# jontio/JAERO

Hardware: AMD Instinct MI355X
Metric: Msamples/s of real 48 kHz PCM through the 10.5 kbps OQPSK demodulator hot path (higher is better)
Workload: dtype f64; 1 GPU; 65536-channel-per-GPU synthetic 48 kHz 10.5 kbps OQPSK continuous (BASELINE configs[2] shape, scaled to 65536 channels per GPU = one wavefront of 64 channels per SIMD), 4096-sample writes, coarse 2^14 FFT every 4096 samples, AFC off, EbNo meters on, Eb/N0 10.0 dB, per-channel carrier (8000 +- 100 Hz), bits, noise, symbol phase; 42 untimed pre-roll steps (the last 18 resident and back to back with ; channels_per_gpu=65536, total_channels=65536, chunk=4096, ebno_meters=True, preroll_steps=42, timing_phases=32, hbm_bytes_per_resident_channel=2256640, resident_channels_max=137027, ranks=1, control_plane=none (single rank), sustain_steps=18

## Files before the change

### jaero_amd/csrc/jaero_device.h

```cpp
#pragma once
#include <hip/hip_runtime.h>
#include <stdint.h>
#include "jd_libm.h"

#define JD_WTSIZE 19999
#define JD_WAVE 64

enum
{
    S_M2_PTR, S_M2_STEP, S_M2_FREQ,
    S_MC_PTR, S_MC_STEP, S_MC_FREQ,
    S_ST_PTR, S_ST_STEP, S_ST_FREQ, S_ST_LAST,
    S_AGC_SUM,
    S_EB_ESUM, S_EB_E2SUM, S_EB_EBNO,
    S_D1,
    S_D41_1, S_D41_2, S_D41_3,
    S_D42_1, S_D42_2, S_D42_3,
    S_D8_1, S_D8_2,
    S_RES_X1, S_RES_X2, S_RES_Y1, S_RES_Y2,
    S_LF_X1, S_LF_X2, S_LF_Y1, S_LF_Y2,
    S_SIG2L_RE, S_SIG2L_IM, S_PTD_RE, S_PTD_IM,
    S_MARG_SUM, S_PM_SUM, S_MSEMA_SUM, S_MSE,
    S_DIFF_LAST,
    S_LOCKINGBW, S_THRESH,
// ... 411 lines not shown
                if (((hx & 0xfffffu) | (unsigned)__double2loint(x)) != 0) return x + x;
                return (xsb == 0) ? x : -1.0;
            }
            if (x > o_threshold) return huge * huge;
        }
        if (xsb != 0 && x + tiny < 0.0) return tiny - one;
    }
    if (hx > 0x3fd62e42u)
    {
        if (hx < 0x3FF0A2B2u)
        {
            if (xsb == 0) { hi = x - ln2_hi; lo = ln2_lo; k = 1; }
            else { hi = x + ln2_hi; lo = -ln2_lo; k = -1; }
        }
        else
        {
            k = (int)(invln2 * x + ((xsb == 0) ? 0.5 : -0.5));
            t = k;
            hi = x - t * ln2_hi;
            lo = t * ln2_lo;
        }
        x = hi - lo;
        c = (hi - x) - lo;
    }
    else if (hx < 0x3c900000u) return x;
    else k = 0;
    hfx = 0.5 * x;
    hxs = x * hfx;
    {
        const double R1 = one + hxs * Q1, h2 = hxs * hxs;
        const double R2 = Q2 + hxs * Q3, h4 = h2 * h2;
        const double R3 = Q4 + hxs * Q5;
        r1 = R1 + h2 * R2 + h4 * R3;
    }
    t = 3.0 - r1 * hfx;
    e = hxs * ((r1 - t) / (6.0 - x * t));
    if (k == 0) return x - (x * e - hxs);
    e = (x * (e - c) - c);
    e -= hxs;
    if (k == -1) return 0.5 * (x - e) - 0.5;
    if (k == 1)
    {
        if (x < -0.25) return -2.0 * (e - (x + 0.5));
        return one + 2.0 * (x - e);
    }
    if (k <= -2 || k > 56)
    {
        y = one - (e - x);
        y = jd_with_hi(y, __double2hiint(y) + (k << 20));
        return y - one;
    }
    if (k < 20)
    {
        t = jd_with_hi(one, 0x3ff00000 - (0x200000 >> k));
        y = t - (e - x);
        y = jd_with_hi(y, __double2hiint(y) + (k << 20));
    }
    else
    {
        t = jd_with_hi(one, (0x3ff - k) << 20);
        y = x - (e + t);
        y += one;
        y = jd_with_hi(y, __double2hiint(y) + (k << 20));
    }
    return y;
}
__device__ __noinline__ double jd_tanh_full(double x)
{
    const double one = 1.0, two = 2.0, tiny = 1.0e-300;
    double t, z;
    const int jx = __double2hiint(x);
    const int ix = jx & 0x7fffffff;
    if (ix >= 0x7ff00000) return (jx >= 0) ? one / x + one : one / x - one;
    if (ix < 0x40360000)
    {
        if ((ix | __double2loint(x)) == 0) return x;
        if (ix < 0x3c800000) return x * (one + x);
        const bool big = ix >= 0x3ff00000;
        const double ax2 = two * fabs(x);
        t = jd_expm1(big ? ax2 : -ax2);
        const double q = (big ? two : t) / (t + two);
        z = big ? one - q : -q;
    }
    else z = one - tiny;
    return (jx >= 0) ? z : -z;
}

__device__ __forceinline__ double jd_tanh(double xin)
{
    const double one = 1.0, two = 2.0, ln2_hi = 6.93147180369123816490e-01, ln2_lo = 1.90821492927058770002e-10,
                 invln2 = 1.44269504088896338700e+00, Q1 = -3.33333333333331316428e-02, Q2 = 1.58730158725481460165e-03,
                 Q3 = -7.93650757867487942473e-05, Q4 = 4.00821782732936239552e-06, Q5 = -2.01099218183624371326e-07;
    const int jx = __double2hiint(xin), ix = jx & 0x7fffffff;
    if (!(ix >= 0x3c800000 && ix < 0x401a0000)) return jd_tanh_full(xin);
    const bool big = ix >= 0x3ff00000;
    const double ax2 = two * fabs(xin);
    double x = big ? ax2 : -ax2;
    const unsigned hx = (unsigned)__double2hiint(x) & 0x7fffffffu;
    const int k = (hx > 0x3fd62e42u) ? (int)(invln2 * x + (big ? 0.5 : -0.5)) : 0;
    const double tk = (double)k;
    const double hi = x - tk * ln2_hi, lo = tk * ln2_lo;
    x = hi - lo;
    const double c = (hi - x) - lo;
    const double hfx = 0.5 * x, hxs = x * hfx;
    const double R1 = one + hxs * Q1, h2 = hxs * hxs, R2 = Q2 + hxs * Q3, h4 = h2 * h2, R3 = Q4 + hxs * Q5;
    const double r1 = R1 + h2 * R2 + h4 * R3;
    const double t3 = 3.0 - r1 * hfx;
    const double e = hxs * jd_div(r1 - t3, 6.0 - x * t3);
    const double r_k0 = x - (x * e - hxs);
    double e2 = (x * (e - c) - c);
    e2 -= hxs;
    const double r_m1 = 0.5 * (x - e2) - 0.5;
    double yn = one - (e2 - x);
    yn = jd_with_hi(yn, __double2hiint(yn) + (k << 20));
    const double r_neg = yn - one;
    const double tm = jd_with_hi(one, 0x3ff00000 - (0x200000 >> (k & 31)));
    double ym = tm - (e2 - x);
    ym = jd_with_hi(ym, __double2hiint(ym) + (k << 20));
    const double t = (k == 0) ? r_k0 : (k == -1) ? r_m1 : (k <= -2) ? r_neg : ym;
    const double q = jd_div(big ? two : t, t + two);
    const double z = big ? one - q : -q;
    return (jx >= 0) ? z : -z;
}

__device__ __forceinline__ double jd_log10(double x)
{
#pragma clang fp contract(fast)
    int e;
    double m = frexp(x, &e);
    if (m < 0.70710678118654752440) { m *= 2.0; e -= 1; }
    const double d = m + 1.0, n = m - 1.0;
    double r = __builtin_amdgcn_rcp(d);
    r = fma(fma(-d, r, 1.0), r, r);
    r = fma(fma(-d, r, 1.0), r, r);
    const double s = n * r;
    const double sl = fma(-d, s, n) * r;
    const double z = s * s;
    double q = 1.0 / 19.0;
    q = fma(q, z, 1.0 / 17.0);
    q = fma(q, z, 1.0 / 15.0);
    q = fma(q, z, 1.0 / 13.0);
    q = fma(q, z, 1.0 / 11.0);
    q = fma(q, z, 1.0 / 9.0);
    q = fma(q, z, 1.0 / 7.0);
    q = fma(q, z, 1.0 / 5.0);
    q = fma(q, z, 1.0 / 3.0);
    const double t = fma(s * z, q, sl);
    const double kh = 0x1.bcb7b1526e50ep-1, kl = 0x1.95355baaafad3p-56;
    const double ch = 0x1.34413509f79ffp-2, cl = -0x1.9dc1da994fd21p-59;
    const double u = fma(s, kh, fma(t, kh, s * kl));
    const double ef = (double)e;
    return fma(ef, ch, fma(ef, cl, u));
}
```

### jaero_amd/csrc/k_coarse6.h

```cpp
#pragma once
#include "k_coarse2.h"

#ifndef C4_TABN
#define C4_TABN 3584
#endif
#define C6_FENCE __builtin_amdgcn_sched_barrier(0)
__device__ __forceinline__ double2 c6_sq(const double2 a)
{
#pragma clang fp contract(fast)
    return make_double2(a.x * a.x - a.y * a.y, 2.0 * (a.x * a.y));
}

#ifndef C6_TRACE
#define C6_TRACE(i)
#endif

template <int CTRL, int ROWMASK>
__device__ __forceinline__ void c6_argmax_step(double &bv, int &bi)
{
    const int lo = __builtin_amdgcn_update_dpp(__double2loint(bv), __double2loint(bv), CTRL, ROWMASK, 0xf, false);
    const int hi = __builtin_amdgcn_update_dpp(__double2hiint(bv), __double2hiint(bv), CTRL, ROWMASK, 0xf, false);
    const int oi = __builtin_amdgcn_update_dpp(bi, bi, CTRL, ROWMASK, 0xf, false);
    const double ov = __hiloint2double(hi, lo);
    const bool take = (oi >= 0) & ((bi < 0) | (ov > bv) | ((ov == bv) & (oi < bi)));
    bv = take ? ov : bv;
    bi = take ? oi : bi;
}
__device__ __forceinline__ void c6_wave_argmax(double &bv, int &bi)
{
    c6_argmax_step<0xB1, 0xf>(bv, bi);
    c6_argmax_step<0x4E, 0xf>(bv, bi);
    c6_argmax_step<0x141, 0xf>(bv, bi);
    c6_argmax_step<0x140, 0xf>(bv, bi);
    c6_argmax_step<0x142, 0xa>(bv, bi);
    c6_argmax_step<0x143, 0xc>(bv, bi);
    bv = __hiloint2double(__builtin_amdgcn_readlane(__double2hiint(bv), 63), __builtin_amdgcn_readlane(__double2loint(bv), 63));
    bi = __builtin_amdgcn_readlane(bi, 63);
}

#define C6_XCH 16448

__device__ __forceinline__ constexpr int c6_k(int s) { return s < 16 ? 2 * s : 2 * (s - 16) + 1; }

__device__ __forceinline__ void c6_fft32(CV<32> &x)
{
#pragma clang fp contract(fast)
#pragma unroll
    for (int j = 0; j < 16; j++)
    {
        const double ar = x.r[j], ai = x.i[j], br = x.r[j + 16], bi = x.i[j + 16];
        x.r[j] = ar + br; x.i[j] = ai + bi;
        double dr = ar - br, di = ai - bi;
        cmul_w64(dr, di, 2 * j);
        x.r[j + 16] = dr; x.i[j + 16] = di;
    }
    C6_FENCE;
#pragma unroll
    for (int h = 0; h < 2; h++)
    {
        CV<16> in, out;
#pragma unroll
        for (int j = 0; j < 16; j++) { in.r[j] = x.r[16 * h + j]; in.i[j] = x.i[16 * h + j]; }
        regfft<16>(in, out);
#pragma unroll
        for (int j = 0; j < 16; j++) { x.r[16 * h + j] = out.r[j]; x.i[16 * h + j] = out.i[j]; }
        C6_FENCE;
    }
}

__device__ __forceinline__ void c6_twiddle32(CV<32> &x, const double2 p1)
{
#pragma clang fp contract(fast)
    auto app = [&](int slot, const double2 w) __attribute__((always_inline)) {
        const double r = x.r[slot] * w.x - x.i[slot] * w.y, i = x.r[slot] * w.y + x.i[slot] * w.x;
        x.r[slot] = r; x.i[slot] = i;
    };
    const double2 p2 = c6_sq(p1);
    double2 e = p2;
    app(16, p1);
#pragma unroll
    for (int j = 1; j < 16; j++)
    {
        app(j, e);
        app(16 + j, cmul2(e, p1));
        if (j < 15) e = cmul2(e, p2);
    }
}

#ifndef C6_ABSORB
#define C6_ABSORB 2
#endif

__device__ __forceinline__ constexpr int c6_brev(int v, int bits)
{
    int r = 0;
    for (int i = 0; i < bits; i++) r |= ((v >> i) & 1) << (bits - 1 - i);
    return r;
}

__device__ __forceinline__ double2 c6_root_mul(const double2 p, int idx)
{
#pragma clang fp contract(fast)
    const int e = idx & 15;
    double2 r = p;
    if (e != 0)
    {
        const double wr = jd_w64r(e), wi = jd_w64i(e);
        r = make_double2(p.x * wr - p.y * wi, p.x * wi + p.y * wr);
    }
    return (idx & 16) ? make_double2(r.y, -r.x) : r;
}

__device__ __forceinline__ void c6_ratio_powers(const double2 r, double2 (&P)[5])
{
    P[0] = r;
#pragma unroll
    for (int i = 1; i < 5; i++) P[i] = c6_sq(P[i - 1]);
}

template <int L, int OFF, int Z>
__device__ __forceinline__ void c6_afft(CV<32> &x, const double2 (&P)[5])
{
    constexpr int LG = L == 32 ? 5 : 4, S = 64 / L;
#pragma unroll
    for (int lv = 0; lv < LG; lv++)
    {
#pragma unroll
        for (int b = 0; b < (1 << lv); b++)
        {
            const int half = L >> (lv + 1);
            const double2 w = c6_root_mul(P[LG - 1 - lv], half * (S * c6_brev(b, lv) + Z));
#pragma unroll
            for (int j = 0; j < half; j++)
            {
                const int ia = OFF + 2 * half * b + j, ib = ia + half;
                const double ar = x.r[ia], ai = x.i[ia], br = x.r[ib], bi = x.i[ib];
                const double ur = __builtin_fma(-w.y, bi, __builtin_fma(w.x, br, ar));
                const double ui = __builtin_fma(w.x, bi, __builtin_fma(w.y, br, ai));
                x.r[ia] = ur; x.i[ia] = ui;
                x.r[ib] = __builtin_fma(2.0, ar, -ur); x.i[ib] = __builtin_fma(2.0, ai, -ui);
            }
        }
        C6_FENCE;
    }
}

__device__ __forceinline__ void c6_afft16x2(CV<32> &x, const double2 r)
{
    double2 P[5];
    c6_ratio_powers(r, P);
    c6_afft<16, 0, 0>(x, P);
    c6_afft<16, 16, 2>(x, P);
}

template <int L, int OFF>
__device__ __forceinline__ void c6_twiddle_brev(CV<32> &x, const double2 c, const double2 s)
{
#pragma clang fp contract(fast)
    constexpr int LG = L == 32 ? 5 : 4;
    auto app = [&](int slot, const double2 w) __attribute__((always_inline)) {
        const double r = x.r[slot] * w.x - x.i[slot] * w.y, i = x.r[slot] * w.y + x.i[slot] * w.x;
        x.r[slot] = r; x.i[slot] = i;
    };
    const double2 s2 = c6_sq(s);
    double2 e = c;
#pragma unroll
    for (int j = 0; j < L / 2; j++)
    {
        app(OFF + c6_brev(2 * j, LG), e);
        app(OFF + c6_brev(2 * j + 1, LG), cmul2(e, s));
        if (j < L / 2 - 1) e = cmul2(e, s2);
    }
}

template <bool ABSORBED>
__device__ __forceinline__ void c6_pass3(CV<32> &d, const double2 r)
{
    if constexpr (ABSORBED)
    {
        c6_afft16x2(d, r);
        const CV<32> o = d;
#pragma unroll
        for (int k3 = 0; k3 < 16; k3++)
        {
            d.r[2 * k3] = o.r[c6_brev(k3, 4)]; d.i[2 * k3] = o.i[c6_brev(k3, 4)];
            d.r[2 * k3 + 1] = o.r[16 + c6_brev(k3, 4)]; d.i[2 * k3 + 1] = o.i[16 + c6_brev(k3, 4)];
        }
    }
    else
    {
        CV<16> in, o0, o1;
#pragma unroll
        for (int j = 0; j < 16; j++) { in.r[j] = d.r[j]; in.i[j] = d.i[j]; }
        regfft<16>(in, o0);
        C6_FENCE;
#pragma unroll
        for (int j = 0; j < 16; j++) { in.r[j] = d.r[16 + j]; in.i[j] = d.i[16 + j]; }
        regfft<16>(in, o1);
#pragma unroll
        for (int k3 = 0; k3 < 16; k3++) { d.r[2 * k3] = o0.r[k3]; d.i[2 * k3] = o0.i[k3]; d.r[2 * k3 + 1] = o1.r[k3]; d.i[2 * k3 + 1] = o1.i[k3]; }
    }
}

template <int AB = C6_ABSORB>
__device__ __forceinline__ void wg_fft14_e32(CV<32> &d, double *xch, const double2 *__restrict__ tw, int t)
{
#pragma clang fp contract(fast)
    const int k1u = t >> 4, n3 = t & 15, odd = k1u & 1;
    const double2 st1 = tw[AB ? 16 * k1u : t], st2 = tw[AB == 2 ? t : 32 * n3];
    double2 st3 = st2;
    if constexpr (AB == 1) st3 = tw[k1u * n3];
    const int e1w0 = t, e1w1 = (t + 16) & 511;
    const int e1r = k1u * 512 + odd * 16 + n3;
    const int e1rw = e1r + 496 - 512 * odd;
    const int e2w = k1u + n3 * 513;
    const int e2r = t;
    auto k2of = [](int s) __attribute__((always_inline)) { return AB ? c6_brev(s, 5) : c6_k(s); };

    c6_fft32(d);
    if constexpr (AB == 0) c6_twiddle32(d, st1);
    C6_FENCE;
    jd_lds_barrier();
#pragma unroll
    for (int s = 0; s < 32; s++) xch[c6_k(s) * 512 + ((c6_k(s) & 1) ? e1w1 : e1w0)] = d.r[s];
    jd_lds_barrier();
#pragma unroll
    for (int m = 0; m < 32; m++) d.r[m] = xch[(m < 31 ? e1r + 16 * m : e1rw)];
    jd_lds_barrier();
#pragma unroll
    for (int s = 0; s < 32; s++) xch[c6_k(s) * 512 + ((c6_k(s) & 1) ? e1w1 : e1w0)] = d.i[s];
    jd_lds_barrier();
#pragma unroll
    for (int m = 0; m < 32; m++) d.i[m] = xch[(m < 31 ? e1r + 16 * m : e1rw)];
    C6_FENCE;
    if constexpr (AB == 0)
    {
        c6_fft32(d);
        c6_twiddle32(d, st2);
    }
    else
    {
        double2 P[5];
        c6_ratio_powers(st1, P);
        c6_afft<32, 0, 0>(d, P);
        if constexpr (AB == 1) c6_twiddle_brev<32, 0>(d, st3, st2);
    }
    C6_FENCE;
    jd_lds_barrier();
#pragma unroll
    for (int s = 0; s < 32; s++) xch[e2w + (k2of(s) & 15) * 32 + (k2of(s) >> 4) * 8208] = d.r[s];
    jd_lds_barrier();
#pragma unroll
    for (int m = 0; m < 32; m++) d.r[m] = xch[e2r + (m & 15) * 513 + (m >> 4) * 8208];
    jd_lds_barrier();
#pragma unroll
    for (int s = 0; s < 32; s++) xch[e2w + (k2of(s) & 15) * 32 + (k2of(s) >> 4) * 8208] = d.i[s];
    jd_lds_barrier();
#pragma unroll
    for (int m = 0; m < 32; m++) d.i[m] = xch[e2r + (m & 15) * 513 + (m >> 4) * 8208];
    C6_FENCE;
    c6_pass3<AB == 2>(d, st2);
}


#define C6_XCH13 8208
template <int AB = C6_ABSORB>
__device__ __forceinline__ void wg_fft13_e32(CV<32> &d, double *xch, const double2 *__restrict__ tw, int t)
{
#pragma clang fp contract(fast)
    const int k1a = t >> 4, n3 = t & 15;
    const double2 st1 = tw[AB ? 16 * k1a : t], st2 = tw[AB == 2 ? t : 32 * n3];
    const int e1r = k1a * 256 + n3;
    const int e2w = k1a + 513 * n3;
    auto k2of = [](int s) __attribute__((always_inline)) { return AB ? c6_brev(s & 15, 4) : (s & 15); };
    c6_fft32(d);
    if constexpr (AB == 0) c6_twiddle32(d, st1);
    C6_FENCE;
    jd_lds_barrier();
#pragma unroll
    for (int s = 0; s < 32; s++) (xch + c6_k(s) * 256)[t] = d.r[s];
    jd_lds_barrier();
#pragma unroll
    for (int m = 0; m < 32; m++) d.r[m] = (xch + (m >> 4) * 4096 + (m & 15) * 16)[e1r];
    jd_lds_barrier();
#pragma unroll
    for (int s = 0; s < 32; s++) (xch + c6_k(s) * 256)[t] = d.i[s];
    jd_lds_barrier();
#pragma unroll
    for (int m = 0; m < 32; m++) d.i[m] = (xch + (m >> 4) * 4096 + (m & 15) * 16)[e1r];
    C6_FENCE;
    if constexpr (AB == 0)
    {
#pragma unroll
        for (int g2 = 0; g2 < 2; g2++)
        {
            CV<16> in, out;
#pragma unroll
            for (int j = 0; j < 16; j++) { in.r[j] = d.r[16 * g2 + j]; in.i[j] = d.i[16 * g2 + j]; }
            regfft<16>(in, out);
            c4_twiddle16(out, st2);
#pragma unroll
            for (int j = 0; j < 16; j++) { d.r[16 * g2 + j] = out.r[j]; d.i[16 * g2 + j] = out.i[j]; }
            C6_FENCE;
        }
    }
    else
    {
        c6_afft16x2(d, st1);
        if constexpr (AB == 1)
        {
            c6_twiddle_brev<16, 0>(d, tw[n3 * k1a], st2);
            c6_twiddle_brev<16, 16>(d, tw[n3 * (k1a + 16)], st2);
        }
        C6_FENCE;
    }
    jd_lds_barrier();
#pragma unroll
    for (int s = 0; s < 32; s++) (xch + (s >> 4) * 16 + k2of(s) * 32)[e2w] = d.r[s];
    jd_lds_barrier();
#pragma unroll
    for (int m = 0; m < 32; m++) d.r[m] = (xch + (m >> 4) * 256 + (m & 15) * 513)[t];
    jd_lds_barrier();
#pragma unroll
    for (int s = 0; s < 32; s++) (xch + (s >> 4) * 16 + k2of(s) * 32)[e2w] = d.i[s];
    jd_lds_barrier();
#pragma unroll
    for (int m = 0; m < 32; m++) d.i[m] = (xch + (m >> 4) * 256 + (m & 15) * 513)[t];
    C6_FENCE;
    c6_pass3<AB == 2>(d, st2);
}

template <int LOG2N>
__device__ __forceinline__ void c6_fft(CV<32> &d, double *xch, const double2 *__restrict__ tw, int t)
{
    int tt = t;
    asm volatile("" : "+v"(tt));
    if constexpr (LOG2N == 14) wg_fft14_e32(d, xch, tw, tt);
    else wg_fft13_e32(d, xch, tw, tt);
}

__device__ __noinline__ void c6_build_window(double *wt, int startbin, int t, int nthreads)
{
    for (int i = t; i <= startbin + 1; i += nthreads)
    {
        const double c = cos(M_PI_2 * ((double)i) / ((double)startbin));
        wt[i] = (i == 0) ? 1.0 : ((i <= startbin) ? c * c : 0.0);
    }
}

template <bool W8400, int LOG2N = 14>
__device__ __forceinline__ void coarse6_body(const JGeom g, const JPtrs p, const int *__restrict__ chan_list, int nlist, const double2 *__restrict__ tw)
{
    constexpr int N = 1 << LOG2N;
    constexpr int E = 32;
    constexpr int NT = N / E;
    constexpr int XCH = LOG2N == 14 ? C6_XCH : C6_XCH13;
    extern __shared__ __attribute__((aligned(16))) double xch[];
    __shared__ double red_val[NT / 64];
    __shared__ int red_idx[NT / 64];
    const int t0 = threadIdx.x;
    const int nchp = g.nchp;
    int tab_startbin = -1;

    CV<E> d;
    int ch_next = ((int)blockIdx.x < nlist) ? (chan_list ? jd_sload(chan_list + blockIdx.x) : (int)blockIdx.x) : 0;
    int bp_next = jd_sload(p.I + (size_t)I_BB_PTR * nchp + ch_next);
    for (int li = blockIdx.x; li < nlist; li += gridDim.x)
    {
        int t = t0;
        asm volatile("" : "+v"(t));
        const int ch = ch_next, bb_ptr = bp_next;
        const double2 *__restrict__ ring = p.bbring + (size_t)ch * N;
        const int ln = li + (int)gridDim.x;
        const bool has_next = ln < nlist;
        if (has_next)
        {
            ch_next = chan_list ? jd_sload(chan_list + ln) : ln;
            bp_next = jd_sload(p.I + (size_t)I_BB_PTR * nchp + ch_next);
        }
        const double lockingbw = jd_sload(p.S + (size_t)S_LOCKINGBW * nchp + ch);
        double fs_l = g.Fs;
        asm volatile("" : "+s"(fs_l));
        int startbin, expectedpeakbin;
        {
            const double hzperbin = fs_l * (1.0 / ((double)N));
            startbin = __builtin_amdgcn_readfirstlane((int)fmax(round(lockingbw / hzperbin), 1.0));
            expectedpeakbin = __builtin_amdgcn_readfirstlane((int)round(g.fb / (2.0 * hzperbin)));
        }
        const int stopbin = N - startbin;
        double *__restrict__ y = p.y + (size_t)ch * N;

        if (li == (int)blockIdx.x)
        {
#pragma unroll
            for (int s = 0; s < E; s++)
            {
                const double2 v = ring[(bb_ptr + s * NT + t) & (N - 1)];
                d.r[s] = v.x; d.i[s] = v.y;
            }
        }
        C6_TRACE(0);
        c6_fft<LOG2N>(d, xch, tw, t);
        C6_TRACE(1);
        if constexpr (W8400)
        {
            const bool persistent = startbin < C4_TABN - 1;
            double *wt = persistent ? xch + XCH : xch;
            if (!persistent || startbin != tab_startbin)
            {
                jd_lds_barrier();
                c6_build_window(wt, startbin, t, NT);
                jd_lds_barrier();
                if (persistent) tab_startbin = startbin;
            }
#pragma unroll
            for (int s0 = 0; s0 < E; s0 += 8)
            {
#pragma unroll
                for (int s = s0; s < s0 + 8; s++)
                {
                    const int k = s * NT + t;
                    const int i = (k <= N / 2) ? k : N - k;
                    const double w = wt[i <= startbin ? i : startbin + 1];
                    const double re = d.r[s] * w, im = d.i[s] * w;
                    d.r[s] = im; d.i[s] = re;
                }
                C6_FENCE;
            }
            if (!persistent) jd_lds_barrier();
        }
        else
        {
#pragma unroll
            for (int s = 0; s < E; s++)
            {
                const int k = s * NT + t;
                const bool z = (k >= startbin) && (k <= stopbin);
                const double re = z ? 0.0 : d.r[s], im = z ? 0.0 : d.i[s];
                d.r[s] = im; d.i[s] = re;
            }
        }
        c6_fft<LOG2N>(d, xch, tw, t);
        C6_TRACE(2);
#pragma unroll
        for (int s = 0; s < E; s++)
        {
            const double re = d.i[s], im = d.r[s];
            d.r[s] = re * re - im * im;
            d.i[s] = re * im + im * re;
        }
        c6_fft<LOG2N>(d, xch, tw, t);
        C6_TRACE(3);
        jd_lds_barrier();
        CoarseSlotState cst;
        {
            double yv[E];
#pragma unroll
            for (int s = 0; s < E; s++) d.r[s] = d.r[s] * d.r[s] + d.i[s] * d.i[s];
            C6_FENCE;
#pragma unroll
            for (int s = 0; s < E; s++) yv[s] = __builtin_nontemporal_load((y + ((s * NT) ^ (N / 2))) + t);
            C6_FENCE;
            cst = coarse_slot_load_v(g, p, ch);
            int bpn = bp_next, chn = ch_next, tp = t;
            asm volatile("" : "+v"(bpn), "+v"(chn), "+v"(tp));
            typedef double c6_v2 __attribute__((ext_vector_type(2)));
            const c6_v2 *__restrict__ ringn = (const c6_v2 *)(p.bbring + (size_t)chn * N);
            const int toffp = bpn + tp;
#pragma unroll
            for (int s = 0; s < E; s++)
            {
                const int ib = (s * NT) ^ (N / 2);
                const double yn = yv[s] * 0.9 + 0.5 * jd_log10(fmax(d.r[s], 1.0));
                __builtin_nontemporal_store(yn, (y + ib) + t);
                (xch + ib)[t] = yn;
                {
                    const c6_v2 v = __builtin_nontemporal_load(ringn + ((toffp + s * NT) & (N - 1)));
                    d.r[s] = v.x; d.i[s] = v.y;
                }
                if ((s & 3) == 3) C6_FENCE;
            }
            C6_TRACE(4);
            jd_lds_barrier();
            C6_TRACE(5);
        }
        C6_TRACE(6);
        double fs_e = g.Fs;
        asm volatile("" : "+s"(fs_e));
        const double hzperbin = fs_e * (1.0 / ((double)N));
        const int i0 = __builtin_amdgcn_readfirstlane((int)round((-lockingbw / hzperbin) + ((double)(N / 2))));
        const int i1 = __builtin_amdgcn_readfirstlane((int)round((lockingbw / hzperbin) + ((double)(N / 2))));
        double best = 0;
        int besti = -1;
        const bool fold_inside = (i0 - expectedpeakbin - 1 >= 0) && (i1 + expectedpeakbin < N) && (i0 >= 0);
        if (fold_inside)
        {
            const int nblk = (i1 - i0 + 4 * NT - 1) / (4 * NT);
            for (int b = 0; b < nblk; b++)
            {
                double val[4];
#pragma unroll
                for (int u = 0; u < 4; u++)
                {
                    const int i = i0 + t + (4 * b + u) * NT;
                    const int ic = i < i1 ? i : i1 - 1;
                    const double *lo = xch + (ic - expectedpeakbin), *hi = xch + (ic + expectedpeakbin);
                    double v = 0;
                    v += (lo[1] + hi[-1]);
                    v += (lo[0] + hi[0]);
                    v += (lo[-1] + hi[1]);
                    val[u] = v;
                }
#pragma unroll
                for (int u = 0; u < 4; u++)
                {
                    const int i = i0 + t + (4 * b + u) * NT;
                    const bool take = (i < i1) & (val[u] > best);
                    best = take ? val[u] : best;
                    besti = take ? i : besti;
                }
            }
        }
        else
        {
            for (int i = i0 + t; i < i1; i += NT)
            {
                if ((i < 0) || (i >= N)) continue;
                double val = 0;
                for (int j = -1; j <= 1; j++)
                {
                    if (((i - expectedpeakbin - j) < 0) || ((i + expectedpeakbin + j) >= N)) continue;
                    val += (xch[i - expectedpeakbin - j] + xch[i + expectedpeakbin + j]);
                }
                if (val > best) { best = val; besti = i; }
            }
        }
        C6_TRACE(7);
        int bigchange;
        {
            double bv = best;
            int bi = besti;
            c6_wave_argmax(bv, bi);
            if ((t & 63) == 0) { red_val[t >> 6] = bv; red_idx[t >> 6] = bi; }
            C6_TRACE(8);
            jd_lds_barrier();
            bv = red_val[0]; bi = red_idx[0];
#pragma unroll
            for (int w = 1; w < NT / 64; w++)
            {
                const double ov = red_val[w];
                const int oi = red_idx[w];
                const bool take = (oi >= 0) & ((bi < 0) | (ov > bv) | ((ov == bv) & (oi < bi)));
                bv = take ? ov : bv;
                bi = take ? oi : bi;
            }
            bigchange = coarse_slot_apply(g, p, ch, cst, (bi >= 0) ? bi : (N / 2), N, hzperbin, lockingbw, t == 0);
            C6_TRACE(9);
        }
        if (bigchange)
        {
            __syncthreads();
            double2 *ringw = p.bbring + (size_t)ch * N;
            for (int i = t; i < N; i += NT) { y[i] = 20; ringw[i] = make_double2(0.0, 0.0); }
        }
        C6_TRACE(10);
    }
}

__global__ __launch_bounds__(C2_THREADS) void k_coarse6(const JGeom g, const JPtrs p, const int *__restrict__ chan_list,
                                                           int nlist, const double2 *__restrict__ tw)
{
    coarse6_body<false>(g, p, chan_list, nlist, tw);
}
__global__ __launch_bounds__(C2_THREADS) void k_coarse6_w8400(const JGeom g, const JPtrs p, const int *__restrict__ chan_list,
                                                                 int nlist, const double2 *__restrict__ tw)
{
    coarse6_body<true>(g, p, chan_list, nlist, tw);
}
__global__ __launch_bounds__(256, 2) void k_coarse6_13(const JGeom g, const JPtrs p, const int *__restrict__ chan_list,
                                                        int nlist, const double2 *__restrict__ tw)
{
    coarse6_body<false, 13>(g, p, chan_list, nlist, tw);
}
```

### jaero_amd/csrc/prims_check.hip

```cpp
#include "jaero_device.h"

#include <vector>

namespace
{
class Bufs
{
  public:
    ~Bufs()
    {
        for (auto &b : bufs_) (void)hipFree(b.dev);
    }
    template <class T> T *in(const T *h, long n) { return (T *)add((void *)h, n * sizeof(T), false); }
    template <class T> T *io(T *h, long n) { return (T *)add((void *)h, n * sizeof(T), true); }
    bool ok() const { return err_ == hipSuccess; }
    int sync()
    {
        if (err_ != hipSuccess) return (int)err_;
        err_ = hipGetLastError();
        if (err_ == hipSuccess) err_ = hipDeviceSynchronize();
        for (auto &b : bufs_)
            if (err_ == hipSuccess && b.back) err_ = hipMemcpy(b.host, b.dev, b.bytes, hipMemcpyDeviceToHost);
        return (int)err_;
    }

  private:
    struct B { void *host, *dev; size_t bytes; bool back; };
    void *add(void *h, size_t bytes, bool back)
    {
        void *d = nullptr;
        if (err_ == hipSuccess) err_ = hipMalloc(&d, bytes ? bytes : 8);
        if (err_ == hipSuccess) bufs_.push_back({h, d, bytes, back});
        if (err_ == hipSuccess && bytes) err_ = hipMemcpy(d, h, bytes, hipMemcpyHostToDevice);
        return d;
    }
    std::vector<B> bufs_;
    hipError_t err_ = hipSuccess;
};
constexpr int TPB = 256;
inline unsigned nblocks(long n) { return (unsigned)((n + TPB - 1) / TPB); }
}

#define JP_IDX const long i = (long)blockIdx.x * TPB + threadIdx.x

__global__ void __launch_bounds__(TPB) k_jp_atan2(const double *y, const double *x, double *o, long n, unsigned long long mask)
{
    const int lane = threadIdx.x & 63;
    const JdAtanLane T = jd_atan_lane_table(lane);
    JP_IDX;
    if (i < n && (mask >> lane & 1)) o[i] = jd_atan2(y[i], x[i], T);
}
__global__ void __launch_bounds__(TPB) k_jp_hypot(const double *x, const double *y, double *o, long n)
{
    JP_IDX;
    if (i < n) o[i] = jd_hypot(x[i], y[i]);
}
__global__ void __launch_bounds__(TPB) k_jp_div(const double *a, const double *b, double *o, double *o_ieee, long n)
{
    JP_IDX;
    if (i < n) { o[i] = jd_div(a[i], b[i]); o_ieee[i] = a[i] / b[i]; }
}

__global__ void __launch_bounds__(TPB) k_jp_div_const(const double *x, double *o, double *o_ieee, long n, double d, double rd)
{
    JP_IDX;
    if (i < n) { o[i] = jd_div_const(x[i], d, rd); o_ieee[i] = x[i] / d; }
}
__global__ void __launch_bounds__(TPB) k_jp_tanh(const double *x, double *o, long n)
{
    JP_IDX;
    if (i < n) o[i] = jd_tanh(x[i]);
}
__global__ void __launch_bounds__(TPB) k_jp_tanh_full(const double *x, double *o, long n)
{
    JP_IDX;
    if (i < n) o[i] = jd_tanh_full(x[i]);
}
__global__ void __launch_bounds__(TPB) k_jp_expm1(const double *x, double *o, long n)
{
    JP_IDX;
    if (i < n) o[i] = jd_expm1(x[i]);
}
__global__ void __launch_bounds__(TPB) k_jp_log10(const double *x, double *o, long n)
{
    JP_IDX;
    if (i < n) o[i] = jd_log10(x[i]);
}
__global__ void __launch_bounds__(TPB) k_jp_qround(const double *x, int *o, long n)
{
    JP_IDX;
    if (i < n) o[i] = jd_qround(x[i]);
}
__global__ void __launch_bounds__(TPB) k_jp_softbit(const double *x, int *o, long n)
{
    JP_IDX;
    if (i < n) o[i] = jd_softbit(x[i]);
}
__global__ void __launch_bounds__(TPB) k_jp_cisidx(const double *x, int *o, long n)
{
    JP_IDX;
    if (i < n) o[i] = jd_cisidx(x[i]);
}
__global__ void __launch_bounds__(TPB) k_jp_wt_next(double *ptr, double *step, long n)
{
    JP_IDX;
    if (i < n) { double p = ptr[i], s = step[i]; jd_wt_next(p, s); ptr[i] = p; step[i] = s; }
}
__global__ void __launch_bounds__(TPB) k_jp_wt_setfreq(const double *f, double *freq, double *step, long n, double samplerate)
{
    JP_IDX;
    if (i < n) { double fr, st; jd_wt_setfreq(fr, st, f[i], samplerate); freq[i] = fr; step[i] = st; }
}
__global__ void __launch_bounds__(TPB) k_jp_wt_inc_phase_deg(double *ptr, const double *phase_deg, long n)
{
    JP_IDX;
    if (i < n) { double p = ptr[i]; jd_wt_inc_phase_deg(p, phase_deg[i]); ptr[i] = p; }
}
__global__ void __launch_bounds__(TPB) k_jp_wt_advance_fraction(double *ptr, const double *f, long n)
{
    JP_IDX;
    if (i < n) { double p = ptr[i]; jd_wt_advance_fraction(p, f[i]); ptr[i] = p; }
}
__global__ void __launch_bounds__(TPB) k_jp_wt_passed(const double *last_ptr, const double *ptr, const double *step, const double *fraction_of_wave,
                                                      double *frac, int *passed, long n)
{
    JP_IDX;
    if (i < n) { double fr = frac[i]; passed[i] = jd_wt_passed(last_ptr[i], ptr[i], step[i], fraction_of_wave[i], fr) ? 1 : 0; frac[i] = fr; }
}
__global__ void __launch_bounds__(TPB) k_jp_fb_wt_setfreq(const double *f, double *freq, double *step, long n, double samplerate, double r_samplerate)
{
    JP_IDX;
    if (i < n) { double fr, st; fb_wt_setfreq(fr, st, f[i], samplerate, r_samplerate); freq[i] = fr; step[i] = st; }
}
__global__ void __launch_bounds__(TPB) k_jp_fb_wt_next(double *ptr, double *step, long n)
{
    JP_IDX;
    if (i < n) { double p = ptr[i], s = step[i]; fb_wt_next(p, s); ptr[i] = p; step[i] = s; }
}
__global__ void __launch_bounds__(TPB) k_jp_fb_fmod360(const double *x, double *o, long n)
{
    JP_IDX;
    if (i < n) o[i] = fb_fmod360(x[i]);
}
__global__ void __launch_bounds__(TPB) k_jp_biquad(const double *x, double *st, double *y, long n, int steps, double b0, double b1, double b2,
                                                   double a1, double a2)
{
    JP_IDX;
    if (i >= n) return;
    double x1 = st[i], x2 = st[n + i], y1 = st[2 * n + i], y2 = st[3 * n + i];
    for (int k = 0; k < steps; k++) y[(long)k * n + i] = jd_biquad(x[(long)k * n + i], x1, x2, y1, y2, b0, b1, b2, a1, a2);
    st[i] = x1; st[n + i] = x2; st[2 * n + i] = y1; st[3 * n + i] = y2;
}
__global__ void __launch_bounds__(TPB) k_jp_diff_soft(const double *soft_in, double *diff_last, double *o, long n)
{
    JP_IDX;
    if (i < n) { double d = diff_last[i]; o[i] = jd_diff_soft(soft_in[i], d); diff_last[i] = d; }
}
__global__ void __launch_bounds__(TPB) k_jp_wt_next_symbol(double *ptr, double *step, double *last_ptr, long n)
{
    JP_IDX;
    if (i < n) { double p = ptr[i], s = step[i], l = last_ptr[i]; jd_wt_next_symbol(p, s, l); ptr[i] = p; step[i] = s; last_ptr[i] = l; }
}
__global__ void __launch_bounds__(TPB) k_jp_bd_set_phase_deg(const double *phase_deg, double *ptr, long n)
{
    JP_IDX;
    if (i < n) { double p = ptr[i]; bd_set_phase_deg(p, phase_deg[i]); ptr[i] = p; }
}

template <int FORM, int FIRN, int LDSN, int D, bool FUSED>
__global__ void __launch_bounds__(64) k_jp_fir(const double *taps, const double *tail_re, const double *tail_im, const double *ring_re,
                                               const double *ring_im, JTaps28 tp, double *out_re, double *out_im)
{
    constexpr int TAILN = FIRN - LDSN, TAILA = TAILN > 0 ? TAILN : 1;
    __shared__ double lre[LDSN * 64], lim[LDSN * 64], ltap[FIRN];
    const int lane = threadIdx.x, fir_slot = blockIdx.x;
    for (int s = 0; s < LDSN; s++) { lre[s * 64 + lane] = ring_re[s * 64 + lane]; lim[s * 64 + lane] = ring_im[s * 64 + lane]; }
    for (int k = lane; k < FIRN; k += 64) ltap[k] = taps[k];
    double tre[TAILA], tim[TAILA];
#pragma unroll
    for (int j = 0; j < TAILA; j++) { tre[j] = TAILN > 0 ? tail_re[j * 64 + lane] : 0.0; tim[j] = TAILN > 0 ? tail_im[j * 64 + lane] : 0.0; }
    __syncthreads();
    double ore = 0, oim = 0;
    if constexpr (FORM == 0 && FUSED) jd_fir_sum<FIRN, LDSN, D, true, 0>(JdRingWalk<LDSN>{lre, lim, fir_slot, lane}, ltap, 0, tre, tim, 0.0, 0.0, ore, oim);
    else if constexpr (FORM == 0) jd_fir_eval<FIRN, LDSN, D>(lre, lim, ltap, tre, tim, fir_slot, lane, ore, oim);
    else if constexpr (FORM == 1) jd_fir_eval_sym<FIRN, LDSN, D>(lre, lim, tp, tre, tim, fir_slot, lane, ore, oim);
    else if constexpr (FORM == 2) jd_fir_eval_sym_static<FIRN, LDSN, D>(lre, lim, tp, tre, tim, fir_slot, lane, ore, oim);
    else jd_fir_eval_sym_static_but_last<FIRN, LDSN, D>(lre, lim, tp, tre, tim, fir_slot, lane, ore, oim);
    out_re[fir_slot * 64 + lane] = ore;
    out_im[fir_slot * 64 + lane] = oim;
}
template <int FORM, int FIRN, int LDSN, int D, bool FUSED>
static int run_fir(const double *taps, const double *tail_re, const double *tail_im, const double *ring_re, const double *ring_im, double *out_re,
                   double *out_im)
{
    constexpr int TAILA = FIRN - LDSN > 0 ? FIRN - LDSN : 1;
    JTaps28 tp;
    for (int k = 0; k < 28; k++) tp.t[k] = k < FIRN ? taps[k] : 0.0;
    Bufs b;
    const double *dt = b.in(taps, FIRN), *dtr = b.in(tail_re, TAILA * 64), *dti = b.in(tail_im, TAILA * 64);
    const double *drr = b.in(ring_re, LDSN * 64), *dri = b.in(ring_im, LDSN * 64);
    double *dor = b.io(out_re, LDSN * 64), *doi = b.io(out_im, LDSN * 64);
    if (b.ok()) k_jp_fir<FORM, FIRN, LDSN, D, FUSED><<<LDSN, 64>>>(dt, dtr, dti, drr, dri, tp, dor, doi);
    return b.sync();
}
template <int FIRN, int LDSN, int D, bool FUSED, int T0, int BS>
__global__ void __launch_bounds__(64) k_jp_fir_blocks(const double *taps, const double *tail_re, const double *tail_im, const double *ring_re,
                                                      const double *ring_im, const double *start_re, const double *start_im, double *out_re, double *out_im)
{
    constexpr int TAILN = FIRN - T0 - LDSN, TAILA = TAILN > 0 ? TAILN : 1;
    extern __shared__ __attribute__((aligned(16))) double lds[];
    double *lre = lds, *lim = lds + LDSN * 64, *ltap = lds + 2 * LDSN * 64;
    const int lane = threadIdx.x, fir_slot = blockIdx.x;
    for (int s = 0; s < LDSN; s++) { lre[s * 64 + lane] = ring_re[s * 64 + lane]; lim[s * 64 + lane] = ring_im[s * 64 + lane]; }
    for (int k = lane; k < FIRN; k += 64) ltap[k] = taps[k];
    double tre[TAILA], tim[TAILA];
#pragma unroll
    for (int j = 0; j < TAILA; j++) { tre[j] = TAILN > 0 ? tail_re[j * 64 + lane] : 0.0; tim[j] = TAILN > 0 ? tail_im[j * 64 + lane] : 0.0; }
    __syncthreads();
    double ore = 0, oim = 0;
    jd_fir_sum_blocks<FIRN, LDSN, D, FUSED, T0, BS>(lre, ltap, jd_vzero(), tre, tim, fir_slot, lane, start_re[lane], start_im[lane], ore, oim);
    out_re[fir_slot * 64 + lane] = ore;
    out_im[fir_slot * 64 + lane] = oim;
}
template <int FIRN, int LDSN, int D, bool FUSED, int T0, int BS>
static int run_fir_blocks(const double *taps, const double *tail_re, const double *tail_im, const double *ring_re, const double *ring_im,
                          const double *start_re, const double *start_im, double *out_re, double *out_im)
{
    constexpr int TAILA = FIRN - T0 - LDSN > 0 ? FIRN - T0 - LDSN : 1, LDS_BYTES = (2 * LDSN * 64 + FIRN) * (int)sizeof(double);
    const auto kernel = k_jp_fir_blocks<FIRN, LDSN, D, FUSED, T0, BS>;
    const hipError_t e = hipFuncSetAttribute((const void *)kernel, hipFuncAttributeMaxDynamicSharedMemorySize, LDS_BYTES);
    if (e != hipSuccess) return (int)e;
    Bufs b;
    const double *dt = b.in(taps, FIRN), *dtr = b.in(tail_re, TAILA * 64), *dti = b.in(tail_im, TAILA * 64);
    const double *drr = b.in(ring_re, LDSN * 64), *dri = b.in(ring_im, LDSN * 64), *dsr = b.in(start_re, 64), *dsi = b.in(start_im, 64);
    double *dor = b.io(out_re, LDSN * 64), *doi = b.io(out_im, LDSN * 64);
    if (b.ok()) kernel<<<LDSN, 64, LDS_BYTES>>>(dt, dtr, dti, drr, dri, dsr, dsi, dor, doi);
    return b.sync();
}

extern "C" {
int jp_atan2(const double *y, const double *x, double *o, long n, unsigned long long mask)
{
    Bufs b;
    const double *dy = b.in(y, n), *dx = b.in(x, n);
    double *d = b.io(o, n);
    if (b.ok() && n > 0) k_jp_atan2<<<nblocks(n), TPB>>>(dy, dx, d, n, mask);
    return b.sync();
}
#define JP_2IN_1OUT(NAME, T)                                                                                                                         \
    int NAME(const double *a, const double *c, T *o, long n)                                                                                         \
    {                                                                                                                                                \
        Bufs b;                                                                                                                                      \
        const double *da = b.in(a, n), *dc = b.in(c, n);                                                                                             \
        T *d = b.io(o, n);                                                                                                                           \
        if (b.ok() && n > 0) k_##NAME<<<nblocks(n), TPB>>>(da, dc, d, n);                                                                            \
        return b.sync();                                                                                                                             \
    }
#define JP_1IN_1OUT(NAME, T)                                                                                                                         \
    int NAME(const double *a, T *o, long n)                                                                                                          \
    {                                                                                                                                                \
        Bufs b;                                                                                                                                      \
        const double *da = b.in(a, n);                                                                                                               \
        T *d = b.io(o, n);                                                                                                                           \
        if (b.ok() && n > 0) k_##NAME<<<nblocks(n), TPB>>>(da, d, n);                                                                                \
        return b.sync();                                                                                                                             \
    }
JP_2IN_1OUT(jp_hypot, double)
JP_1IN_1OUT(jp_tanh, double)
JP_1IN_1OUT(jp_tanh_full, double)
JP_1IN_1OUT(jp_expm1, double)
JP_1IN_1OUT(jp_log10, double)
JP_1IN_1OUT(jp_qround, int)
JP_1IN_1OUT(jp_softbit, int)
JP_1IN_1OUT(jp_cisidx, int)
JP_1IN_1OUT(jp_fb_fmod360, double)
int jp_div(const double *a, const double *bb, double *o, double *o_ieee, long n)
{
    Bufs b;
    const double *da = b.in(a, n), *db = b.in(bb, n);
    double *d = b.io(o, n), *di = b.io(o_ieee, n);
    if (b.ok() && n > 0) k_jp_div<<<nblocks(n), TPB>>>(da, db, d, di, n);
    return b.sync();
}
int jp_div_const(const double *x, double *o, double *o_ieee, long n, double dd, double rd)
{
    Bufs b;
    const double *dx = b.in(x, n);
    double *d = b.io(o, n), *di = b.io(o_ieee, n);
    if (b.ok() && n > 0) k_jp_div_const<<<nblocks(n), TPB>>>(dx, d, di, n, dd, rd);
    return b.sync();
}
int jp_wt_next(double *ptr, double *step, long n)
{
    Bufs b;
    double *dp = b.io(ptr, n), *ds = b.io(step, n);
    if (b.ok() && n > 0) k_jp_wt_next<<<nblocks(n), TPB>>>(dp, ds, n);
    return b.sync();
}
int jp_fb_wt_next(double *ptr, double *step, long n)
{
    Bufs b;
    double *dp = b.io(ptr, n), *ds = b.io(step, n);
    if (b.ok() && n > 0) k_jp_fb_wt_next<<<nblocks(n), TPB>>>(dp, ds, n);
    return b.sync();
}
int jp_wt_setfreq(const double *f, double *freq, double *step, long n, double samplerate)
{
    Bufs b;
    const double *df = b.in(f, n);
    double *dfr = b.io(freq, n), *ds = b.io(step, n);
    if (b.ok() && n > 0) k_jp_wt_setfreq<<<nblocks(n), TPB>>>(df, dfr, ds, n, samplerate);
    return b.sync();
}
int jp_fb_wt_setfreq(const double *f, double *freq, double *step, long n, double samplerate, double r_samplerate)
{
    Bufs b;
    const double *df = b.in(f, n);
    double *dfr = b.io(freq, n), *ds = b.io(step, n);
    if (b.ok() && n > 0) k_jp_fb_wt_setfreq<<<nblocks(n), TPB>>>(df, dfr, ds, n, samplerate, r_samplerate);
    return b.sync();
}
int jp_wt_inc_phase_deg(double *ptr, const double *phase_deg, long n)
{
    Bufs b;
    double *dp = b.io(ptr, n);
    const double *dph = b.in(phase_deg, n);
    if (b.ok() && n > 0) k_jp_wt_inc_phase_deg<<<nblocks(n), TPB>>>(dp, dph, n);
    return b.sync();
}
int jp_wt_advance_fraction(double *ptr, const double *f, long n)
{
    Bufs b;
    double *dp = b.io(ptr, n);
    const double *df = b.in(f, n);
    if (b.ok() && n > 0) k_jp_wt_advance_fraction<<<nblocks(n), TPB>>>(dp, df, n);
    return b.sync();
}
int jp_wt_passed(const double *last_ptr, const double *ptr, const double *step, const double *fraction_of_wave, double *frac, int *passed, long n)
{
    Bufs b;
    const double *dl = b.in(last_ptr, n), *dp = b.in(ptr, n), *ds = b.in(step, n), *dw = b.in(fraction_of_wave, n);
    double *dfr = b.io(frac, n);
    int *dpa = b.io(passed, n);
    if (b.ok() && n > 0) k_jp_wt_passed<<<nblocks(n), TPB>>>(dl, dp, ds, dw, dfr, dpa, n);
    return b.sync();
}
int jp_biquad(const double *x, double *st, double *y, long n, int steps, double b0, double b1, double b2, double a1, double a2)
{
    Bufs b;
    const double *dx = b.in(x, n * steps);
    double *ds = b.io(st, 4 * n), *dy = b.io(y, n * steps);
    if (b.ok() && n > 0) k_jp_biquad<<<nblocks(n), TPB>>>(dx, ds, dy, n, steps, b0, b1, b2, a1, a2);
    return b.sync();
}
int jp_diff_soft(const double *soft_in, double *diff_last, double *o, long n)
{
    Bufs b;
    const double *dsi = b.in(soft_in, n);
    double *dd = b.io(diff_last, n), *d = b.io(o, n);
    if (b.ok() && n > 0) k_jp_diff_soft<<<nblocks(n), TPB>>>(dsi, dd, d, n);
    return b.sync();
}
int jp_wt_next_symbol(double *ptr, double *step, double *last_ptr, long n)
{
    Bufs b;
    double *dp = b.io(ptr, n), *ds = b.io(step, n), *dl = b.io(last_ptr, n);
    if (b.ok() && n > 0) k_jp_wt_next_symbol<<<nblocks(n), TPB>>>(dp, ds, dl, n);
    return b.sync();
}
int jp_bd_set_phase_deg(const double *phase_deg, double *ptr, long n)
{
    Bufs b;
    const double *dph = b.in(phase_deg, n);
    double *dp = b.io(ptr, n);
    if (b.ok() && n > 0) k_jp_bd_set_phase_deg<<<nblocks(n), TPB>>>(dph, dp, n);
    return b.sync();
}

#define JP_FIR(NAME, FORM, FIRN, LDSN, D, FUSED)                                                                                                     \
    int NAME(const double *taps, const double *tail_re, const double *tail_im, const double *ring_re, const double *ring_im, double *out_re,        \
             double *out_im)                                                                                                                         \
    {                                                                                                                                                \
        return run_fir<FORM, FIRN, LDSN, D, FUSED>(taps, tail_re, tail_im, ring_re, ring_im, out_re, out_im);                                       \
    }
JP_FIR(jp_fir_eval_40_24_8, 0, 40, 24, 8, false)
JP_FIR(jp_fir_eval_20_12_8, 0, 20, 12, 8, false)
JP_FIR(jp_fir_eval_fused_55_36_8, 0, 55, 36, 8, true)
JP_FIR(jp_fir_eval_sym_55_36_6, 1, 55, 36, 6, false)
JP_FIR(jp_fir_eval_sym_static_55_36_6, 2, 55, 36, 6, false)
JP_FIR(jp_fir_eval_sym_static_but_last_55_36_6, 3, 55, 36, 6, false)
#define JP_FIR_BLOCKS(NAME, FIRN, LDSN, D, FUSED, T0, BS)                                                                                            \
    int NAME(const double *taps, const double *tail_re, const double *tail_im, const double *ring_re, const double *ring_im,                       \
             const double *start_re, const double *start_im, double *out_re, double *out_im)                                                        \
    {                                                                                                                                                \
        return run_fir_blocks<FIRN, LDSN, D, FUSED, T0, BS>(taps, tail_re, tail_im, ring_re, ring_im, start_re, start_im, out_re, out_im);         \
    }
JP_FIR_BLOCKS(jp_fir_sum_blocks_80_36_8_t32_b4, 80, 36, 8, false, 32, 4)
JP_FIR_BLOCKS(jp_fir_sum_blocks_80_32_8_t18_b4, 80, 32, 8, false, 18, 4)
JP_FIR_BLOCKS(jp_fir_sum_blocks_160_72_8_t64_b4, 160, 72, 8, false, 64, 4)
JP_FIR_BLOCKS(jp_fir_sum_blocks_fused_55_36_8_t0_b6, 55, 36, 8, true, 0, 6)
}
```

Before: 12070 Msamples/s.

## Micro-optimize coarse FFT kernel: fused first pass, cheaper addressing, folded log10 scale

Bundles several small coarse-FFT optimizations, each behind a default-on macro. It replaces the first radix-32 pass with a bit-reversed-output FFT that uses FMA butterflies. Ring-buffer addresses are computed as byte offsets with scalar bases, and the second LDS exchange gets a high-half address base. The band-zero test becomes a single unsigned compare, the squaring and magnitude steps use FMA, and the 0.5 factor is folded into a dedicated log10 routine. The intent is to cut VALU instruction count and address arithmetic in the hot FFT step. The risks are small rounding differences and extra register pressure.

New measurement: 12210 Msamples/s, median of 6. 1.2% higher.

```diff
diff --git a/jaero_amd/csrc/jaero_device.h b/jaero_amd/csrc/jaero_device.h
--- a/jaero_amd/csrc/jaero_device.h
+++ b/jaero_amd/csrc/jaero_device.h
@@ -587,3 +587,33 @@
     const double ef = (double)e;
     return fma(ef, ch, fma(ef, cl, u));
 }
+
+__device__ __forceinline__ double c6_log10_half(double x)
+{
+#pragma clang fp contract(fast)
+    int e;
+    double m = frexp(x, &e);
+    if (m < 0.70710678118654752440) { m *= 2.0; e -= 1; }
+    const double d = m + 1.0, n = m - 1.0;
+    double r = __builtin_amdgcn_rcp(d);
+    r = fma(fma(-d, r, 1.0), r, r);
+    r = fma(fma(-d, r, 1.0), r, r);
+    const double s = n * r;
+    const double sl = fma(-d, s, n) * r;
+    const double z = s * s;
+    double q = 1.0 / 19.0;
+    q = fma(q, z, 1.0 / 17.0);
+    q = fma(q, z, 1.0 / 15.0);
+    q = fma(q, z, 1.0 / 13.0);
+    q = fma(q, z, 1.0 / 11.0);
+    q = fma(q, z, 1.0 / 9.0);
+    q = fma(q, z, 1.0 / 7.0);
+    q = fma(q, z, 1.0 / 5.0);
+    q = fma(q, z, 1.0 / 3.0);
+    const double t = fma(s * z, q, sl);
+    const double kh = 0x1.bcb7b1526e50ep-2, kl = 0x1.95355baaafad3p-57;
+    const double ch = 0x1.34413509f79ffp-3, cl = -0x1.9dc1da994fd21p-60;
+    const double u = fma(s, kh, fma(t, kh, s * kl));
+    const double ef = (double)e;
+    return fma(ef, ch, fma(ef, cl, u));
+}
diff --git a/jaero_amd/csrc/k_coarse6.h b/jaero_amd/csrc/k_coarse6.h
--- a/jaero_amd/csrc/k_coarse6.h
+++ b/jaero_amd/csrc/k_coarse6.h
@@ -91,6 +91,25 @@
 #define C6_ABSORB 2
 #endif
 
+#ifndef C6_HIADDR
+#define C6_HIADDR 1
+#endif
+#ifndef C6_RINGADDR
+#define C6_RINGADDR 1
+#endif
+#ifndef C6_BAND1
+#define C6_BAND1 1
+#endif
+#ifndef C6_SQFMA
+#define C6_SQFMA 1
+#endif
+#ifndef C6_LOGHALF
+#define C6_LOGHALF 1
+#endif
+#ifndef C6_P1FUSED
+#define C6_P1FUSED 1
+#endif
+
 __device__ __forceinline__ constexpr int c6_brev(int v, int bits)
 {
     int r = 0;
@@ -116,6 +135,37 @@
     P[0] = r;
 #pragma unroll
     for (int i = 1; i < 5; i++) P[i] = c6_sq(P[i - 1]);
+}
+
+__device__ __forceinline__ void c6_cfft32(CV<32> &x)
+{
+#pragma unroll
+    for (int lv = 0; lv < 5; lv++)
+    {
+#pragma unroll
+        for (int b = 0; b < (1 << lv); b++)
+        {
+            const int half = 16 >> lv, idx = half * 2 * c6_brev(b, lv), e = idx & 15;
+            const double cr = jd_w64r(e), ci = jd_w64i(e);
+            const double wr = (idx & 16) ? ci : cr, wi = (idx & 16) ? -cr : ci;
+#pragma unroll
+            for (int j = 0; j < half; j++)
+            {
+                const int ia = 2 * half * b + j, ib = ia + half;
+                const double ar = x.r[ia], ai = x.i[ia], br = x.r[ib], bi = x.i[ib];
+                if (idx == 0) { x.r[ia] = ar + br; x.i[ia] = ai + bi; x.r[ib] = ar - br; x.i[ib] = ai - bi; }
+                else if (idx == 16) { x.r[ia] = ar + bi; x.i[ia] = ai - br; x.r[ib] = ar - bi; x.i[ib] = ai + br; }
+                else
+                {
+                    const double ur = __builtin_fma(-wi, bi, __builtin_fma(wr, br, ar));
+                    const double ui = __builtin_fma(wr, bi, __builtin_fma(wi, br, ai));
+                    x.r[ia] = ur; x.i[ia] = ui;
+                    x.r[ib] = __builtin_fma(2.0, ar, -ur); x.i[ib] = __builtin_fma(2.0, ai, -ui);
+                }
+            }
+        }
+        C6_FENCE;
+    }
 }
 
 template <int L, int OFF, int Z>
@@ -202,7 +252,7 @@
     }
 }
 
-template <int AB = C6_ABSORB>
+template <int AB = C6_ABSORB, bool P1 = (AB > 0) && C6_P1FUSED, bool HI = false>
 __device__ __forceinline__ void wg_fft14_e32(CV<32> &d, double *xch, const double2 *__restrict__ tw, int t)
 {
 #pragma clang fp contract(fast)
@@ -216,19 +266,22 @@
     const int e2w = k1u + n3 * 513;
     const int e2r = t;
     auto k2of = [](int s) __attribute__((always_inline)) { return AB ? c6_brev(s, 5) : c6_k(s); };
-
-    c6_fft32(d);
+    auto k1of = [](int s) __attribute__((always_inline)) { return P1 ? c6_brev(s, 5) : c6_k(s); };
+
+    static_assert(!(P1 && AB == 0), "the output twiddle of AB 0 expects split order");
+    if constexpr (P1) c6_cfft32(d);
+    else c6_fft32(d);
     if constexpr (AB == 0) c6_twiddle32(d, st1);
     C6_FENCE;
     jd_lds_barrier();
 #pragma unroll
-    for (int s = 0; s < 32; s++) xch[c6_k(s) * 512 + ((c6_k(s) & 1) ? e1w1 : e1w0)] = d.r[s];
+    for (int s = 0; s < 32; s++) xch[k1of(s) * 512 + ((k1of(s) & 1) ? e1w1 : e1w0)] = d.r[s];
     jd_lds_barrier();
 #pragma unroll
     for (int m = 0; m < 32; m++) d.r[m] = xch[(m < 31 ? e1r + 16 * m : e1rw)];
     jd_lds_barrier();
 #pragma unroll
-    for (int s = 0; s < 32; s++) xch[c6_k(s) * 512 + ((c6_k(s) & 1) ? e1w1 : e1w0)] = d.i[s];
+    for (int s = 0; s < 32; s++) xch[k1of(s) * 512 + ((k1of(s) & 1) ? e1w1 : e1w0)] = d.i[s];
     jd_lds_barrier();
 #pragma unroll
     for (int m = 0; m < 32; m++) d.i[m] = xch[(m < 31 ? e1r + 16 * m : e1rw)];
@@ -246,25 +299,29 @@
         if constexpr (AB == 1) c6_twiddle_brev<32, 0>(d, st3, st2);
     }
     C6_FENCE;
-    jd_lds_barrier();
-#pragma unroll
-    for (int s = 0; s < 32; s++) xch[e2w + (k2of(s) & 15) * 32 + (k2of(s) >> 4) * 8208] = d.r[s];
-    jd_lds_barrier();
-#pragma unroll
-    for (int m = 0; m < 32; m++) d.r[m] = xch[e2r + (m & 15) * 513 + (m >> 4) * 8208];
-    jd_lds_barrier();
-#pragma unroll
-    for (int s = 0; s < 32; s++) xch[e2w + (k2of(s) & 15) * 32 + (k2of(s) >> 4) * 8208] = d.i[s];
-    jd_lds_barrier();
-#pragma unroll
-    for (int m = 0; m < 32; m++) d.i[m] = xch[e2r + (m & 15) * 513 + (m >> 4) * 8208];
+    int e2wh = e2w + (HI ? 8208 : 0), e2rh = e2r + (HI ? 8208 : 0);
+    if constexpr (HI) asm volatile("" : "+v"(e2wh), "+v"(e2rh));
+    constexpr int UP = HI ? 0 : 8208;
+    auto sof = [](int q) __attribute__((always_inline)) { return !HI ? q : AB ? c6_brev(q, 5) : (q & 1) ? 16 + (q >> 1) : (q >> 1); };
+    jd_lds_barrier();
+#pragma unroll
+    for (int q = 0; q < 32; q++) xch[(k2of(sof(q)) >> 4 ? e2wh + UP : e2w) + (k2of(sof(q)) & 15) * 32] = d.r[sof(q)];
+    jd_lds_barrier();
+#pragma unroll
+    for (int m = 0; m < 32; m++) d.r[m] = xch[(m >> 4 ? e2rh + UP : e2r) + (m & 15) * 513];
+    jd_lds_barrier();
+#pragma unroll
+    for (int q = 0; q < 32; q++) xch[(k2of(sof(q)) >> 4 ? e2wh + UP : e2w) + (k2of(sof(q)) & 15) * 32] = d.i[sof(q)];
+    jd_lds_barrier();
+#pragma unroll
+    for (int m = 0; m < 32; m++) d.i[m] = xch[(m >> 4 ? e2rh + UP : e2r) + (m & 15) * 513];
     C6_FENCE;
     c6_pass3<AB == 2>(d, st2);
 }
 
 
 #define C6_XCH13 8208
-template <int AB = C6_ABSORB>
+template <int AB = C6_ABSORB, bool P1 = (AB > 0) && C6_P1FUSED>
 __device__ __forceinline__ void wg_fft13_e32(CV<32> &d, double *xch, const double2 *__restrict__ tw, int t)
 {
 #pragma clang fp contract(fast)
@@ -273,18 +330,21 @@
     const int e1r = k1a * 256 + n3;
     const int e2w = k1a + 513 * n3;
     auto k2of = [](int s) __attribute__((always_inline)) { return AB ? c6_brev(s & 15, 4) : (s & 15); };
-    c6_fft32(d);
+    auto k1of = [](int s) __attribute__((always_inline)) { return P1 ? c6_brev(s, 5) : c6_k(s); };
+    static_assert(!(P1 && AB == 0), "the output twiddle of AB 0 expects split order");
+    if constexpr (P1) c6_cfft32(d);
+    else c6_fft32(d);
     if constexpr (AB == 0) c6_twiddle32(d, st1);
     C6_FENCE;
     jd_lds_barrier();
 #pragma unroll
-    for (int s = 0; s < 32; s++) (xch + c6_k(s) * 256)[t] = d.r[s];
+    for (int s = 0; s < 32; s++) (xch + k1of(s) * 256)[t] = d.r[s];
     jd_lds_barrier();
 #pragma unroll
     for (int m = 0; m < 32; m++) d.r[m] = (xch + (m >> 4) * 4096 + (m & 15) * 16)[e1r];
     jd_lds_barrier();
 #pragma unroll
-    for (int s = 0; s < 32; s++) (xch + c6_k(s) * 256)[t] = d.i[s];
+    for (int s = 0; s < 32; s++) (xch + k1of(s) * 256)[t] = d.i[s];
     jd_lds_barrier();
 #pragma unroll
     for (int m = 0; m < 32; m++) d.i[m] = (xch + (m >> 4) * 4096 + (m & 15) * 16)[e1r];
@@ -335,8 +395,8 @@
 {
     int tt = t;
     asm volatile("" : "+v"(tt));
-    if constexpr (LOG2N == 14) wg_fft14_e32(d, xch, tw, tt);
-    else wg_fft13_e32(d, xch, tw, tt);
+    if constexpr (LOG2N == 14) wg_fft14_e32<C6_ABSORB, (C6_ABSORB > 0) && C6_P1FUSED, C6_HIADDR != 0>(d, xch, tw, tt);
+    else wg_fft13_e32<C6_ABSORB, (C6_ABSORB > 0) && C6_P1FUSED>(d, xch, tw, tt);
 }
 
 __device__ __noinline__ void c6_build_window(double *wt, int startbin, int t, int nthreads)
@@ -392,10 +452,17 @@
 
         if (li == (int)blockIdx.x)
         {
+#if C6_RINGADDR
+            const unsigned boff = ((unsigned)(bb_ptr + t) & (unsigned)(N - 1)) << 4;
+#endif
 #pragma unroll
             for (int s = 0; s < E; s++)
             {
+#if C6_RINGADDR
+                const double2 v = *(const double2 *)((const char *)ring + ((boff + (unsigned)(s * NT * 16)) & (unsigned)(N * 16 - 1)));
+#else
                 const double2 v = ring[(bb_ptr + s * NT + t) & (N - 1)];
+#endif
                 d.r[s] = v.x; d.i[s] = v.y;
             }
         }
@@ -431,11 +498,19 @@
         }
         else
         {
+#if C6_BAND1
+            const int band_lo = stopbin < startbin ? -1 : startbin;
+            const unsigned band_w = stopbin < startbin ? 0u : (unsigned)(stopbin - startbin);
+#endif
 #pragma unroll
             for (int s = 0; s < E; s++)
             {
                 const int k = s * NT + t;
+#if C6_BAND1
+                const bool z = (unsigned)(k - band_lo) <= band_w;
+#else
                 const bool z = (k >= startbin) && (k <= stopbin);
+#endif
                 const double re = z ? 0.0 : d.r[s], im = z ? 0.0 : d.i[s];
                 d.r[s] = im; d.i[s] = re;
             }
@@ -446,8 +521,13 @@
         for (int s = 0; s < E; s++)
         {
             const double re = d.i[s], im = d.r[s];
+#if C6_SQFMA
+            d.r[s] = __builtin_fma(re, re, -(im * im));
+            d.i[s] = 2.0 * (re * im);
+#else
             d.r[s] = re * re - im * im;
             d.i[s] = re * im + im * re;
+#endif
         }
         c6_fft<LOG2N>(d, xch, tw, t);
         C6_TRACE(3);
@@ -456,26 +536,53 @@
         {
             double yv[E];
 #pragma unroll
+#if C6_SQFMA
+            for (int s = 0; s < E; s++) d.r[s] = __builtin_fma(d.r[s], d.r[s], d.i[s] * d.i[s]);
+#else
             for (int s = 0; s < E; s++) d.r[s] = d.r[s] * d.r[s] + d.i[s] * d.i[s];
+#endif
             C6_FENCE;
 #pragma unroll
             for (int s = 0; s < E; s++) yv[s] = __builtin_nontemporal_load((y + ((s * NT) ^ (N / 2))) + t);
             C6_FENCE;
             cst = coarse_slot_load_v(g, p, ch);
             int bpn = bp_next, chn = ch_next, tp = t;
+#if C6_RINGADDR
+            asm volatile("" : "+s"(bpn), "+s"(chn), "+v"(tp));
+#else
             asm volatile("" : "+v"(bpn), "+v"(chn), "+v"(tp));
+#endif
+            int tph = tp + ((C6_HIADDR && LOG2N == 14) ? N / 2 : 0);
+            if constexpr (C6_HIADDR && LOG2N == 14) asm volatile("" : "+v"(tph));
+            constexpr int UPH = (C6_HIADDR && LOG2N == 14) ? N / 2 : 0;
             typedef double c6_v2 __attribute__((ext_vector_type(2)));
+#if !C6_RINGADDR
             const c6_v2 *__restrict__ ringn = (const c6_v2 *)(p.bbring + (size_t)chn * N);
+#endif
+#if C6_RINGADDR
+            const unsigned boffp = ((unsigned)(bpn + tp) & (unsigned)(N - 1)) << 4;
+            const char *__restrict__ ringnb = (const char *)(p.bbring + (size_t)chn * N);
+#else
             const int toffp = bpn + tp;
+#endif
 #pragma unroll
             for (int s = 0; s < E; s++)
             {
                 const int ib = (s * NT) ^ (N / 2);
+#if C6_LOGHALF
+                const double yn = yv[s] * 0.9 + c6_log10_half(fmax(d.r[s], 1.0));
+#else
                 const double yn = yv[s] * 0.9 + 0.5 * jd_log10(fmax(d.r[s], 1.0));
+#endif
                 __builtin_nontemporal_store(yn, (y + ib) + t);
-                (xch + ib)[t] = yn;
+                if (UPH && ib >= UPH) (xch + (ib - UPH))[tph] = yn;
+                else (xch + ib)[t] = yn;
                 {
+#if C6_RINGADDR
+                    const c6_v2 v = __builtin_nontemporal_load((const c6_v2 *)(ringnb + ((boffp + (unsigned)(s * NT * 16)) & (unsigned)(N * 16 - 1))));
+#else
                     const c6_v2 v = __builtin_nontemporal_load(ringn + ((toffp + s * NT) & (N - 1)));
+#endif
                     d.r[s] = v.x; d.i[s] = v.y;
                 }
                 if ((s & 3) == 3) C6_FENCE;
diff --git a/jaero_amd/csrc/prims_check.hip b/jaero_amd/csrc/prims_check.hip
--- a/jaero_amd/csrc/prims_check.hip
+++ b/jaero_amd/csrc/prims_check.hip
@@ -85,6 +85,11 @@
 {
     JP_IDX;
     if (i < n) o[i] = jd_log10(x[i]);
+}
+__global__ void __launch_bounds__(TPB) k_jc_log10_half(const double *x, double *o_half, double *o_product, long n)
+{
+    JP_IDX;
+    if (i < n) { o_half[i] = c6_log10_half(x[i]); o_product[i] = 0.5 * jd_log10(x[i]); }
 }
 __global__ void __launch_bounds__(TPB) k_jp_qround(const double *x, int *o, long n)
 {
@@ -274,6 +279,14 @@
 JP_1IN_1OUT(jp_softbit, int)
 JP_1IN_1OUT(jp_cisidx, int)
 JP_1IN_1OUT(jp_fb_fmod360, double)
+int jc_log10_half(const double *x, double *o_half, double *o_product, long n)
+{
+    Bufs b;
+    const double *dx = b.in(x, n);
+    double *dh = b.io(o_half, n), *dp = b.io(o_product, n);
+    if (b.ok() && n > 0) k_jc_log10_half<<<nblocks(n), TPB>>>(dx, dh, dp, n);
+    return b.sync();
+}
 int jp_div(const double *a, const double *bb, double *o, double *o_ieee, long n)
 {
     Bufs b;
```
